# MarkTakken/kf2vecFSW

Hardware: AMD Instinct MI355X
Metric: Gbases/s k-mer→.kf build at k=7; achieved HBM GB/s vs gfx950 peak (higher is better)
Workload: dtype u32

## Files before the change

kf2vecfsw_amd/csrc/kf_count.hip:

```cpp
#include <hip/hip_runtime.h>
#include <stdint.h>
#include <stdlib.h>

#include <mutex>

#include "kf_front.h"
#include "kf_internal.h"

namespace kf {

constexpr int kBlock = 1024;
constexpr uint32_t kWaveWeights = 20u | 17u << 8 | 11u << 16 | 6u << 24;
constexpr int kXRing = 2;

__device__ __forceinline__ void wg_span(const CountArgs& A, uint64_t& lo, uint64_t& hi) {
    const uint64_t base = A.goff[0];
    const uint64_t total = A.goff[A.n_genomes] - base;
    const uint64_t G = gridDim.x, b = blockIdx.x;
    lo = base + ((total / G * b + (total % G) * b / G) & ~(uint64_t)15);
    hi = (b + 1 == G) ? base + total : base + ((total / G * (b + 1) + (total % G) * (b + 1) / G) & ~(uint64_t)15);
}

template <int K>
struct XL {
    static constexpr uint32_t P = K >= 8 ? (1u << 17) : (2u << (2 * (K + 1)));
    static constexpr uint32_t S = K >= 8 ? (1u << 15) : (2u << (2 * K));
    static constexpr uint32_t bytes = P + S;
};
constexpr int kXChunk = 3 * kChunk;
constexpr uint32_t kHot7 = 0xC000C000u, kStep7 = 0x4000u;
constexpr uint32_t kHot8 = 0xE000E000u, kStep8 = 0x2000u;
constexpr uint32_t kHot6 = 0x80008000u, kStep6 = 0x8000u;
template <int K>
constexpr uint32_t x_hot() { return K >= 8 ? kHot8 : (K == 7 ? kHot7 : kHot6); }
template <int K>
constexpr uint32_t x_step() { return K >= 8 ? kStep8 : (K == 7 ? kStep7 : kStep6); }

__device__ __forceinline__ uint32_t k9_code_of(uint32_t i) { return ((i >> 9) << 10) | (i & 0x1FFu); }

__device__ __forceinline__ uint32_t half_one(uint32_t i) { return 1u << ((i & 1u) << 4); }

template <int B>
__device__ __forceinline__ uint32_t shl1_byte(uint32_t h, uint32_t one) {
    uint32_t r;
    if constexpr (B == 0)
        asm("v_lshlrev_b32_sdwa %0, %1, %2 dst_sel:DWORD dst_unused:UNUSED_PAD src0_sel:BYTE_0 src1_sel:DWORD"
            : "=v"(r) : "v"(h), "v"(one));
    else if constexpr (B == 1)
        asm("v_lshlrev_b32_sdwa %0, %1, %2 dst_sel:DWORD dst_unused:UNUSED_PAD src0_sel:BYTE_1 src1_sel:DWORD"
            : "=v"(r) : "v"(h), "v"(one));
    else if constexpr (B == 2)
        asm("v_lshlrev_b32_sdwa %0, %1, %2 dst_sel:DWORD dst_unused:UNUSED_PAD src0_sel:BYTE_2 src1_sel:DWORD"
            : "=v"(r) : "v"(h), "v"(one));
    else
        asm("v_lshlrev_b32_sdwa %0, %1, %2 dst_sel:DWORD dst_unused:UNUSED_PAD src0_sel:BYTE_3 src1_sel:DWORD"
            : "=v"(r) : "v"(h), "v"(one));
    return r;
}

template <int K>
__device__ __noinline__ void x_drain(uint32_t a, const uint32_t* __restrict__ code2col, uint32_t* gcounts) {
    constexpr uint32_t HOT = x_hot<K>(), STEP = x_step<K>();
    constexpr uint32_t PB = XL<K>::P;
    lds_u32* p = (lds_u32*)(uintptr_t)a;
    uint32_t cur = __hip_atomic_load(p, __ATOMIC_RELAXED, __HIP_MEMORY_SCOPE_WORKGROUP);
    while (cur & HOT) {
        const uint32_t sub = ((cur & (HOT & 0xFFFF0000u)) ? (STEP << 16) : 0u) | ((cur & (HOT & 0xFFFFu)) ? STEP : 0u);
        uint32_t seen = cur;
        if (__hip_atomic_compare_exchange_strong(p, &seen, cur - sub, __ATOMIC_RELAXED, __ATOMIC_RELAXED,
                                                 __HIP_MEMORY_SCOPE_WORKGROUP)) {
            const bool single = a >= PB;
            const uint32_t w = (single ? a - PB : a) >> 2;
            for (uint32_t h = 0; h < 2; ++h) {
                if (!((sub >> (16 * h)) & 0xFFFFu)) continue;
                const uint32_t bin = 2 * w + h;
                if (K == 8 || single) {
                    atomicAdd(gcounts + code2col[bin], STEP);
                } else {
                    atomicAdd(gcounts + code2col[bin >> 2], STEP);
                    atomicAdd(gcounts + code2col[bin & ((1u << (2 * K)) - 1u)], STEP);
                }
            }
            cur -= sub;
        } else {
            cur = seen;
        }
    }
}
template <int K>
__device__ __noinline__ void x_scan_drain(const uint32_t* __restrict__ code2col, uint32_t* gcounts, int lane) {
    constexpr uint32_t HOT = x_hot<K>();
    for (uint32_t w = (uint32_t)lane; w < (K >= 8 ? XL<K>::P : XL<K>::bytes) / 4; w += kWave) {
        const uint32_t v = __hip_atomic_load((lds_u32*)(uintptr_t)(4 * w), __ATOMIC_RELAXED,
                                             __HIP_MEMORY_SCOPE_WORKGROUP);
        if (v & HOT) x_drain<K>(4 * w, code2col, gcounts);
    }
}

constexpr uint32_t kXTabLo = 0x630B6102u;
constexpr uint32_t kXTabHi = 0x67000074u;

struct XBlock {
    uint4 q[3];
};
__device__ __forceinline__ uint32_t x_zmap(uint32_t x, uint32_t e, uint32_t c) {
    uint32_t r;
    asm("v_bitop3_b32 %0, %1, %2, %3 bitop3:0x38" : "=v"(r) : "v"(x), "v"(e), "v"(c));
    return r;
}

constexpr int kXNt = 2;

__device__ __forceinline__ XBlock xc_load(const uint8_t* bytes, uint64_t c0, uint32_t rel, uint32_t end_r, int lane) {
    const uint32_t rec = end_r > rel ? min(end_r - rel, (uint32_t)kXChunk) : 0u;
    const auto rs = __builtin_amdgcn_make_buffer_rsrc((void*)(bytes + c0 + rel), (short)0, (int)rec, 0x00020000);
    XBlock b;
#pragma unroll
    for (int i = 0; i < 3; ++i) {
        const auto v = __builtin_amdgcn_raw_buffer_load_b128(rs, lane * 16 + kChunk * i, 0, kXNt);
        b.q[i] = make_uint4(v[0], v[1], v[2], v[3]);
    }
    return b;
}

__device__ __forceinline__ constexpr uint32_t xc_nl_weights(int i) {
    return (uint32_t)(64 - 8 * i) | (uint32_t)(62 - 8 * i) << 8 | (uint32_t)(60 - 8 * i) << 16 |
           (uint32_t)(58 - 8 * i) << 24;
}
constexpr uint32_t kXcBad = 68u;

struct XcCls {
    uint32_t C, V;
};
__device__ __forceinline__ XcCls xc_cls(const uint4 d) {
    const uint32_t w[4] = {d.x, d.y, d.z, d.w};
    const uint32_t cdf = 0xDFDFDFDFu;
    uint32_t pc[4], z[4];
#pragma unroll
    for (int i = 0; i < 4; ++i) {
        const uint32_t x = w[i];
        const uint32_t e = __builtin_amdgcn_perm(kXTabHi, kXTabLo, x & 0x07070707u);
        z[i] = x_zmap(x, e, cdf);
        pc[i] = __builtin_amdgcn_udot4(x & 0x06060606u, 0x01041040u, (i & 1) ? pc[i - 1] << 8 : 0u, false);
    }
    XcCls r;
    r.C = (pc[1] << 15) | (pc[3] >> 1);
    r.V = __builtin_amdgcn_udot4(z[1], xc_nl_weights(1), __builtin_amdgcn_udot4(z[0], xc_nl_weights(0), 0u, false),
                                 false) +
          __builtin_amdgcn_udot4(z[3], xc_nl_weights(3), __builtin_amdgcn_udot4(z[2], xc_nl_weights(2), 0u, false),
                                 false);
    return r;
}

struct XcWin {
    uint32_t x0, y0, c, nl;
};
__device__ __forceinline__ XcWin xc_window(const XcCls& k, uint32_t rot) {
    uint32_t nl;
    asm("v_min_u32_e32 %0, 1, %1" : "=v"(nl) : "v"(k.V));
    const uint32_t q = min(k.V - 34u, 32u);
    const uint32_t L = (uint32_t)(~0ull << q);
    const uint32_t c = bfi(L, k.C >> 2, k.C);
    const uint32_t pC = wave_shr1(rot, c);
    XcWin x;
    x.x0 = (c << 1) | ((pC << 31) & (0u - nl));
    x.y0 = (c >> 15) | (pC << (17u - 2u * nl));
    x.c = c, x.nl = nl;
    return x;
}
__device__ __forceinline__ uint32_t wave_ror1(uint32_t v) {
    return (uint32_t)__builtin_amdgcn_update_dpp(0, (int)v, 0x13C, 0xF, 0xF, false);
}

template <int K>
__device__ __forceinline__ void xc_pairs(const XcWin& x, uint32_t (&rt)[8]) {
    static_assert(K >= 2 && K <= 7, "pairs of k-mers: k <= 7");
    constexpr uint32_t PM = (1u << (2 * K + 3)) - 4u, SM = (1u << (2 * K + 1)) - 4u;
    const uint32_t one = 1u;
    const uint32_t x0 = x.x0, y0 = x.y0;
    const uint32_t H0 = (x.c << 4) & 0x10101010u, H1 = x.c & 0x10101010u;
#pragma unroll
    for (int j = 0; j < 7; ++j) {
// ... 40 lines not shown
};
__device__ __forceinline__ K9Win k9_window(const XcCls& k, uint32_t rot) {
    uint32_t nl;
    asm("v_min_u32_e32 %0, 1, %1" : "=v"(nl) : "v"(k.V));
    const uint32_t q = min(k.V - 34u, 32u);
    const uint32_t L = (uint32_t)(~0ull << q);
    const uint32_t c = bfi(L, k.C >> 2, k.C);
    const uint32_t pC = wave_shr1(rot, c);
    K9Win x;
    x.c = c, x.nl = nl;
    x.wlo = c | ((pC << 30) & (0u - nl));
    x.whi = pC >> (2u * nl);
    return x;
}

__device__ __forceinline__ uint32_t k9_index(uint32_t wlo, uint32_t whi, uint32_t rlo, uint32_t rhi, int r) {
    const uint32_t y = r < 8 ? wlo >> (2 * r) : __builtin_amdgcn_alignbit(whi, wlo, 2 * r);
    const uint32_t rc = r < 8 ? rhi >> (14 - 2 * r) : __builtin_amdgcn_alignbit(rhi, rlo, 46 - 2 * r);
    const uint32_t c = bfi((uint32_t)__builtin_amdgcn_sbfe((int)y, 9u, 1u), rc, y);
    return bfi(0x1FFu, c, c >> 1) & 0x1FFFFu;
}

__device__ __noinline__ uint32_t k9b_carries(uint32_t wlo, uint32_t whi, const uint32_t* __restrict__ code2col,
                                             uint32_t* gcounts, uint32_t w0, uint32_t w1, uint32_t w2, uint32_t w3,
                                             uint32_t w4, uint32_t w5, uint32_t w6, uint32_t w7, uint32_t w8,
                                             uint32_t w9, uint32_t w10, uint32_t w11, uint32_t w12, uint32_t w13,
                                             uint32_t w14, uint32_t w15) {
    const uint32_t rlo = revpairs(whi) ^ 0xAAAAAAAAu, rhi = revpairs(wlo) ^ 0xAAAAAAAAu;
    const uint32_t rt[16] = {w0, w1, w2, w3, w4, w5, w6, w7, w8, w9, w10, w11, w12, w13, w14, w15};
    uint32_t fixed = 0;
#pragma unroll
    for (int r = 0; r < 16; ++r) {
        const uint32_t w = rt[r], ki = k9_index(wlo, whi, rlo, rhi, r), b = ki & 3u;
        if (((w >> (8 * b)) & 0xFFu) != 0xFFu) continue;
        const uint32_t base = ki & ~3u;
        fixed = 1;
        atomicAdd(gcounts + code2col[k9_code_of(base | b)], 256u);
        for (uint32_t j = b + 1; j < 4; ++j) {
            const uint32_t col = code2col[k9_code_of(base | j)];
            const bool wraps = ((w >> (8 * j)) & 0xFFu) == 0xFFu;
            atomicAdd(gcounts + col, wraps ? 255u : 0xFFFFFFFFu);
            if (!wraps) break;
        }
    }
    return __builtin_amdgcn_ballot_w64(fixed != 0) != 0 ? 1u : 0u;
}

template <bool DENSE>
__device__ __forceinline__ uint32_t k9b_region(uint32_t wlo, uint32_t whi, uint32_t R, const CountArgs& A,
                                               uint32_t* gcounts) {
    const uint32_t rlo = revpairs(whi) ^ 0xAAAAAAAAu, rhi = revpairs(wlo) ^ 0xAAAAAAAAu;
    uint32_t rt[16];
#pragma unroll
    for (int r = 0; r < 16; ++r) {
        const uint32_t ki = k9_index(wlo, whi, rlo, rhi, r);
        rt[r] = 0;
        const bool v = (DENSE && r < 15) || ((R >> r) & 1u);
        if (v) rt[r] = lds_add_rtn(ki & 0x1FFFCu, 1u << ((ki << 3) & 24u));
    }
    uint32_t acc = 0;
#pragma unroll
    for (int r = 0; r < 16; ++r) acc |= ~(rt[r] + 0x01010101u) & rt[r];
    if (__builtin_amdgcn_ballot_w64((acc & 0x80808080u) != 0) == 0) return 0;
    return k9b_carries(wlo, whi, A.code2col, gcounts, rt[0], rt[1], rt[2], rt[3], rt[4], rt[5], rt[6], rt[7], rt[8],
                       rt[9], rt[10], rt[11], rt[12], rt[13], rt[14], rt[15]);
}

template <int K>
__device__ __forceinline__ bool xc_fast(const XBlock& d, const CountArgs& A, int lane, uint32_t& carry,
                                        uint32_t* gcounts, uint32_t& lane_total, uint32_t& drained) {
    constexpr uint32_t HOT = x_hot<K>();
    constexpr uint32_t TM = (1u << (2 * (K - 1))) - 1u;
    const XcCls k0 = xc_cls(d.q[0]), k1 = xc_cls(d.q[1]), k2 = xc_cls(d.q[2]);
    carry = __builtin_amdgcn_readfirstlane(carry);
    if (t_n(carry) < (uint32_t)(K - 1) || __builtin_amdgcn_ballot_w64(max(max(k0.V, k1.V), k2.V) >= kXcBad) != 0)
        return false;
    if constexpr (K == 9) {
        const K9Win x0 = k9_window(k0, t_codes(carry));
        uint32_t f = k9b_region<true>(x0.wlo, x0.whi, 0xFFFFu >> x0.nl, A, gcounts);
        const K9Win x1 = k9_window(k1, wave_ror1(x0.c));
        f |= k9b_region<true>(x1.wlo, x1.whi, 0xFFFFu >> x1.nl, A, gcounts);
        const K9Win x2 = k9_window(k2, wave_ror1(x1.c));
        f |= k9b_region<true>(x2.wlo, x2.whi, 0xFFFFu >> x2.nl, A, gcounts);
        lane_total -= x0.nl + x1.nl + x2.nl;
        carry = tail_pack((uint32_t)__builtin_amdgcn_readlane((int)x2.c, kWave - 1) & TM, 31u, 31u);
        drained |= f;
        return true;
    }
    uint32_t o = 0;
    const XcWin x0 = xc_window(k0, t_codes(carry));
    const XcWin x1 = xc_window(k1, wave_ror1(x0.c));
    const XcWin x2 = xc_window(k2, wave_ror1(x1.c));
    if constexpr (K <= 7) {
        const XcWin* xs[3] = {&x0, &x1, &x2};
#pragma unroll
        for (int i = 0; i < 3; ++i) {
            uint32_t r[8];
            xc_pairs<K>(*xs[i], r);
#pragma unroll
            for (int j = 0; j < 8; j += 4) o |= r[j] | r[j + 1] | r[j + 2] | r[j + 3];
        }
    } else {
        const XcWin* xs[3] = {&x0, &x1, &x2};
#pragma unroll
        for (int i = 0; i < 3; ++i) {
            uint32_t r[16];
            xc_wins8(*xs[i], r);
#pragma unroll
            for (int j = 0; j < 16; j += 4) o |= r[j] | r[j + 1] | r[j + 2] | r[j + 3];
        }
    }
    lane_total -= x0.nl + x1.nl + x2.nl;
    carry = tail_pack((uint32_t)__builtin_amdgcn_readlane((int)x2.c, kWave - 1) & TM, 31u, 31u);
    if (__builtin_amdgcn_ballot_w64((o & HOT) != 0) != 0) {
        x_scan_drain<K>(A.code2col, gcounts, lane);
        drained = 1;
    }
    return true;
}

template <int K, bool MASKED>
__device__ __forceinline__ uint32_t x_singles(const uint4 d, const CountArgs& A, uint64_t chunk, int lane,
                                              const ChunkMask& m, uint64_t iv0, uint32_t carry, uint32_t* gcounts,
                                              uint32_t& lane_total, uint32_t& drained) {
    constexpr uint32_t HOT = x_hot<K>();
    uint32_t C, V, EN, ne, own;
    front_end<K, MASKED, false>(d, A, chunk, lane, m, iv0, C, V, EN, ne, own);
    const Windows win = windows<K, MASKED>(C, V, EN, ne, carry, lane);
    const uint32_t wlo = win.wlo, whi = win.whi, R = win.R;
    if constexpr (K == 9) {
        drained |= k9b_region<false>(wlo, whi, R, A, gcounts);
        lane_total += (uint32_t)__builtin_popcount(R);
        return win.next;
    }
    const uint32_t wv[4] = {wlo, __builtin_amdgcn_alignbit(whi, wlo, 8), __builtin_amdgcn_alignbit(whi, wlo, 16),
                            __builtin_amdgcn_alignbit(whi, wlo, 24)};
    uint32_t o = 0;
#pragma unroll
    for (int r = 0; r < 16; ++r) {
        const int fo = (2 * r) & ~7;
        const uint32_t y = __builtin_amdgcn_ubfe(wv[fo >> 3], 2 * r - fo, 2 * K);
        o |= lds_add_rtn((K == 8 ? 0u : XL<K>::P) + ((y >> 1) << 2), ((R >> r) & 1u) * half_one(y));
    }
    if (__builtin_amdgcn_ballot_w64((o & HOT) != 0) != 0) {
        x_scan_drain<K>(A.code2col, gcounts, lane);
        drained = 1;
    }
    lane_total += (uint32_t)__builtin_popcount(R);
    return win.next;
}

template <int K>
__device__ __forceinline__ uint32_t x_range(const CountArgs& A, int32_t g, uint64_t glo, uint64_t ghi, uint64_t lo,
                                            uint64_t hi, int lane, uint32_t& drained) {
    if (lo >= hi) return 0;
    uint32_t* gcounts = A.counts + (uint64_t)g * A.nbins;
    Range rg;
    rg.init(glo, ghi, lo, hi);
    auto load = [&](uint32_t r) {
        return xc_load(A.bytes, rg.c0, r, rg.end_r, lane);
    };
    static_assert(kXRing == 2, "two-deep register ring");
    XBlock buf[K == 9 ? 1 : kXRing];
    XBlock b0, b1;
    if constexpr (K == 9) {
        b0 = load(0);
        b1 = load(kXChunk);
    } else {
#pragma unroll
        for (int j = 0; j < kXRing; ++j) buf[j] = load(j * kXChunk);
    }
    const uint32_t nx = (rg.nch + 2) / 3;
    rg.warm16<K>(A, lane);
    __builtin_amdgcn_s_setprio(0);
    uint32_t carry = rg.carry;
    uint32_t rel = 0;
    const ChunkMask m = rg.mask();
    uint32_t lane_total = 0;
    uint32_t nfast = 0;
    auto step = [&](const XBlock& bf) {
        bool fast = !rg.masked_span(A, rel, kXChunk);
        if (fast)
            fast = xc_fast<K>(bf, A, lane, carry, gcounts, lane_total, drained);
        nfast += fast ? 1u : 0u;
        if (!fast) {
            const bool m0 = rg.masked(A, rel);
            const uint64_t iv0 = rg.iv;
            const bool m1 = rg.masked(A, rel + kChunk);
            const uint64_t iv1 = rg.iv;
            const bool m2 = rg.masked(A, rel + 2 * kChunk);
#pragma unroll
            for (int h = 0; h < 3; ++h) {
                const uint32_t r = rel + h * kChunk;
                if (h > 0 && r >= rg.nch * kChunk) break;
                const bool mh = h == 0 ? m0 : (h == 1 ? m1 : m2);
                const uint64_t ivh = h == 0 ? iv0 : (h == 1 ? iv1 : rg.iv);
                const uint4 hb = bf.q[h];
                if (mh)
                    carry = x_singles<K, true>(hb, A, rg.c0 + r, lane, m, ivh, carry, gcounts, lane_total, drained);
                else
                    carry = x_singles<K, false>(hb, A, rg.c0 + r, lane, m, ivh, carry, gcounts, lane_total, drained);
            }
        }
        rel += kXChunk;
    };
    if constexpr (K == 9) {
        for (uint32_t i = 0; i + 2 <= nx; i += 2) {
            step(b0);
            b0 = load(rel + kXChunk);
            step(b1);
            b1 = load(rel + kXChunk);
        }
        if (nx & 1u) step(b0);
    } else {
        for (uint32_t i = 0; i + kXRing <= nx; i += kXRing) {
#pragma unroll
            for (int j = 0; j < kXRing; ++j) {
                step(buf[j]);
                buf[j] = load(rel + (kXRing - 1) * kXChunk);
            }
        }
        const uint32_t rem = nx % kXRing;
#pragma unroll
        for (int j = 0; j < kXRing - 1; ++j)
            if (rem > (uint32_t)j) step(buf[j]);
    }
    return lane_total + 48u * nfast;
}

__device__ __forceinline__ uint32_t f_swz(uint32_t y) { return y ^ (((y >> 8) & 15u) << 1); }
__device__ __forceinline__ uint32_t u16sum2(uint32_t w) { return (w & 0xFFFFu) + (w >> 16); }

__device__ __forceinline__ void pair_f_sums(const uint32_t* hist, int tid, uint32_t (&F)[16]) {
    const uint4* h4 = (const uint4*)hist;
#pragma unroll
    for (int i = 0; i < 8; ++i) {
        const uint4 w = h4[i * 1024 + tid];
        F[2 * i] = u16sum2(w.x) + u16sum2(w.y);
        F[2 * i + 1] = u16sum2(w.z) + u16sum2(w.w);
#pragma unroll
        for (int a = 0; a < 4; ++a) {
            const uint32_t v = hist[a * 8192 + i * 1024 + tid];
            F[2 * i] += v & 0xFFFFu;
            F[2 * i + 1] += v >> 16;
        }
    }
}

template <int K>
__device__ __forceinline__ void pair_f_sums_small(const uint32_t* hist, int tid,
                                                  uint32_t (&F)[((1u << (2 * K)) + kBlock - 1) / kBlock]) {
    constexpr uint32_t NY = 1u << (2 * K), NM = (NY + kBlock - 1) / kBlock;
#pragma unroll
    for (uint32_t m = 0; m < NM; ++m) {
        const uint32_t y = (uint32_t)tid + kBlock * m;
        F[m] = 0;
        if (y < NY) {
            const uint32_t sh = (y & 1u) << 4;
            uint32_t f = u16sum2(hist[2 * y]) + u16sum2(hist[2 * y + 1]);
#pragma unroll
            for (uint32_t a = 0; a < 4; ++a) f += (hist[a * (NY / 2) + (y >> 1)] >> sh) & 0xFFFFu;
            f += (hist[XL<K>::P / 4 + (y >> 1)] >> sh) & 0xFFFFu;
            F[m] = f;
        }
    }
}

template <int K>
__global__ void __launch_bounds__(kBlock) __attribute__((amdgpu_waves_per_eu(4, 4))) k1x_kernel(CountArgs A) {
    static_assert(K >= 2 && K <= 9, "K1x serves k = 2 .. 9 (k = 9: K9b byte counters)");
    extern __shared__ __attribute__((aligned(16))) uint32_t hist[];
    const int tid = threadIdx.x;
    const int lane = tid & (kWave - 1);
    const int wave = __builtin_amdgcn_readfirstlane(tid >> 6);
    {
        uint4* h4 = (uint4*)hist;
        for (uint32_t i = tid; i < XL<K>::bytes / 16; i += kBlock) h4[i] = make_uint4(0u, 0u, 0u, 0u);
    }
    __syncthreads();
    if ((uint32_t)(uintptr_t)(lds_u32*)hist != 0u) __builtin_trap();
    uint64_t span_lo, span_hi;
    wg_span(A, span_lo, span_hi);
    if (span_lo >= span_hi) return;
    int32_t g = (int32_t)wave_upper_bound((uint64_t)A.n_genomes, span_lo, lane,
                                          [&](uint64_t i) { return A.goff[i + 1]; });
    const uint32_t fr_lo = wave_frac((uint32_t)wave, kWaveWeights), fr_hi = wave_frac((uint32_t)wave + 1, kWaveWeights);
    for (; g < A.n_genomes; ++g) {
        __builtin_amdgcn_s_setprio(3);
        const uint64_t glo = A.goff[g], ghi = A.goff[g + 1];
        if (glo >= span_hi) break;
        const uint64_t plo = max(glo, span_lo), phi = min(ghi, span_hi);
        if (phi <= plo) continue;
        const uint64_t lo = split_at_frac(plo, phi, fr_lo), hi = split_at_frac(plo, phi, fr_hi);
        uint32_t drained = 0;
        unsigned long long s = x_range<K>(A, g, glo, ghi, lo, hi, lane, drained);
        uint32_t* gc = A.counts + (uint64_t)g * A.nbins;
        const bool whole = plo == glo && phi == ghi && !(A.flags & KF_ACCUMULATE);
        if constexpr (K == 9) {
            lds_barrier();
            if (lane == 0) hist[XL<K>::P / 4 + wave] = drained;
            lds_barrier();
            const uint4* fl = (const uint4*)(hist + XL<K>::P / 4);
            const uint4 f0 = fl[0], f1 = fl[1], f2 = fl[2], f3 = fl[3];
            const bool any_fix = (f0.x | f0.y | f0.z | f0.w | f1.x | f1.y | f1.z | f1.w | f2.x | f2.y | f2.z |
                                  f2.w | f3.x | f3.y | f3.z | f3.w) != 0;
            const uint8_t* hb = (const uint8_t*)hist;
            for (uint32_t c0 = (uint32_t)tid; c0 < (1u << 17); c0 += 4 * kBlock) {
                uint32_t rep[4];
#pragma unroll
                for (int j = 0; j < 4; ++j) rep[j] = A.col2rep[c0 + j * kBlock];
#pragma unroll
                for (int j = 0; j < 4; ++j) {
                    const uint32_t c = (rep[j] & 0x200u) ? kf_revcomp<9>(rep[j]) : rep[j];
                    const uint32_t v = hb[((c >> 1) & 0x1FE00u) | (c & 0x1FFu)];
                    if (whole && !any_fix)
                        __builtin_nontemporal_store(v, gc + c0 + j * kBlock);
                    else if (v)
                        __hip_atomic_fetch_add(gc + c0 + j * kBlock, v, __ATOMIC_RELAXED, __HIP_MEMORY_SCOPE_AGENT);
                }
            }
            lds_barrier();
            uint4* h4 = (uint4*)hist;
            for (uint32_t i = tid; i < XL<K>::bytes / 16; i += kBlock) h4[i] = make_uint4(0u, 0u, 0u, 0u);
        } else if constexpr (K == 8) {
            lds_barrier();
            if (lane == 0) hist[XL<K>::P / 4 + wave] = drained;
            lds_barrier();
            const uint4* fl = (const uint4*)(hist + XL<K>::P / 4);
            const uint4 f0 = fl[0], f1 = fl[1], f2 = fl[2], f3 = fl[3];
            const bool any_drain = (f0.x | f0.y | f0.z | f0.w | f1.x | f1.y | f1.z | f1.w | f2.x | f2.y | f2.z |
                                    f2.w | f3.x | f3.y | f3.z | f3.w) != 0;
            for (uint32_t col = tid; col < A.nbins; col += kBlock) {
                const uint32_t y = A.col2rep[col], rc = kf_revcomp<8>(y);
                uint32_t v = (hist[y >> 1] >> ((y & 1u) << 4)) & 0xFFFFu;
                if (rc != y) v += (hist[rc >> 1] >> ((rc & 1u) << 4)) & 0xFFFFu;
                if (whole && !any_drain)
                    gc[col] = v;
                else if (v)
                    __hip_atomic_fetch_add(gc + col, v, __ATOMIC_RELAXED, __HIP_MEMORY_SCOPE_AGENT);
            }
            lds_barrier();
            uint4* h4 = (uint4*)hist;
            for (uint32_t i = tid; i < XL<K>::bytes / 16; i += kBlock) h4[i] = make_uint4(0u, 0u, 0u, 0u);
        } else if constexpr (K <= 6) {
            constexpr uint32_t NY = 1u << (2 * K), NM = (NY + kBlock - 1) / kBlock;
            constexpr uint32_t NCOL = (NY + (K % 2 == 0 ? (1u << K) : 0u)) / 2, NC = (NCOL + kBlock - 1) / kBlock;
            uint32_t rep[NC];
#pragma unroll
            for (uint32_t c = 0; c < NC; ++c) {
                const uint32_t col = (uint32_t)tid + c * kBlock;
                rep[c] = col < NCOL ? A.col2rep[col] : 0u;
            }
            lds_barrier();
            uint32_t F[NM];
            pair_f_sums_small<K>(hist, tid, F);
            lds_barrier();
#pragma unroll
            for (uint32_t m = 0; m < NM; ++m) {
                const uint32_t y = (uint32_t)tid + kBlock * m;
                if (y < NY) hist[f_swz(y)] = F[m];
            }
            if (lane == 0) hist[NY + wave] = drained;
            lds_barrier();
            const uint4* fl = (const uint4*)(hist + NY);
            const uint4 f0 = fl[0], f1 = fl[1], f2 = fl[2], f3 = fl[3];
            const bool any_drain = (f0.x | f0.y | f0.z | f0.w | f1.x | f1.y | f1.z | f1.w | f2.x | f2.y | f2.z | f2.w |
                                    f3.x | f3.y | f3.z | f3.w) != 0;
            uint32_t cv[NC];
#pragma unroll
            for (uint32_t c = 0; c < NC; ++c) {
                const uint32_t y = rep[c], rc = kf_revcomp<K>(y);
                cv[c] = hist[f_swz(y)] + (rc != y ? hist[f_swz(rc)] : 0u);
            }
            lds_barrier();
            uint4* h4 = (uint4*)hist;
            for (uint32_t i = tid; i < XL<K>::bytes / 16; i += kBlock) h4[i] = make_uint4(0u, 0u, 0u, 0u);
#pragma unroll
            for (uint32_t c = 0; c < NC; ++c) {
                const uint32_t col = (uint32_t)tid + c * kBlock;
                if (col >= NCOL) continue;
                if (whole && !any_drain)
                    __builtin_nontemporal_store(cv[c], gc + col);
                else if (cv[c])
                    __hip_atomic_fetch_add(gc + col, cv[c], __ATOMIC_RELAXED, __HIP_MEMORY_SCOPE_AGENT);
            }
        } else {
            uint32_t rep[8];
            if (whole) {
                const uint4 r0 = *(const uint4*)(A.col2rep + 4 * tid), r1 = *(const uint4*)(A.col2rep + 4096 + 4 * tid);
                rep[0] = r0.x, rep[1] = r0.y, rep[2] = r0.z, rep[3] = r0.w;
                rep[4] = r1.x, rep[5] = r1.y, rep[6] = r1.z, rep[7] = r1.w;
            } else {
#pragma unroll
                for (int c = 0; c < 8; ++c) rep[c] = A.col2rep[tid + c * kBlock];
            }
            lds_barrier();
            uint32_t F[16];
            pair_f_sums(hist, tid, F);
#pragma unroll
            for (int i = 0; i < 8; ++i) {
                const uint32_t v = hist[XL<K>::P / 4 + i * 1024 + tid];
                F[2 * i] += v & 0xFFFFu;
                F[2 * i + 1] += v >> 16;
            }
            lds_barrier();
#pragma unroll
            for (int i = 0; i < 8; ++i) *(uint2*)(hist + f_swz(i * 2048 + 2 * tid)) = make_uint2(F[2 * i], F[2 * i + 1]);
            if (lane == 0) hist[16384 + wave] = drained;
            lds_barrier();
            const uint4* fl = (const uint4*)(hist + 16384);
            const uint4 f0 = fl[0], f1 = fl[1], f2 = fl[2], f3 = fl[3];
            const bool any_drain = (f0.x | f0.y | f0.z | f0.w | f1.x | f1.y | f1.z | f1.w | f2.x | f2.y | f2.z | f2.w |
                                    f3.x | f3.y | f3.z | f3.w) != 0;
            uint32_t cv[8];
#pragma unroll
            for (int c = 0; c < 8; ++c) {
                const uint32_t y = rep[c], rc = kf_revcomp<7>(y);
                cv[c] = hist[f_swz(y)] + hist[f_swz(rc)];
            }
            lds_barrier();
            uint4* h4 = (uint4*)hist;
            for (uint32_t i = tid; i < XL<K>::bytes / 16; i += kBlock) h4[i] = make_uint4(0u, 0u, 0u, 0u);
            if (whole && !any_drain) {
                typedef unsigned int v4u_t __attribute__((ext_vector_type(4)));
                __builtin_nontemporal_store(v4u_t{cv[0], cv[1], cv[2], cv[3]}, (v4u_t*)(gc + 4 * tid));
                __builtin_nontemporal_store(v4u_t{cv[4], cv[5], cv[6], cv[7]}, (v4u_t*)(gc + 4096 + 4 * tid));
            } else {
#pragma unroll
                for (int c = 0; c < 8; ++c) {
                    const uint32_t col = whole ? (c >> 2) * 4096 + 4 * tid + (c & 3) : tid + c * kBlock;
                    if (cv[c]) __hip_atomic_fetch_add(gc + col, cv[c], __ATOMIC_RELAXED, __HIP_MEMORY_SCOPE_AGENT);
                }
            }
        }
        s = wave_sum(s);
        if (lane == 0 && s) atomicAdd(A.totals + g, s);
        lds_barrier();
    }
}

__device__ __forceinline__ uint64_t splitmix64(uint64_t x) {
    x += 0x9E3779B97F4A7C15ull;
    x = (x ^ (x >> 30)) * 0xBF58476D1CE4E5B9ull;
    x = (x ^ (x >> 27)) * 0x94D049BB133111EBull;
    return x ^ (x >> 31);
}

__device__ __forceinline__ bool in_nrun(uint64_t key, uint64_t i, uint64_t n_period) {
    if (!n_period) return false;
    uint64_t b = i >> 12;
    for (int d = 0; d < 2; ++d) {
        if (d == 1) {
            if (b == 0) break;
            b -= 1;
        }
        const uint64_t h = splitmix64((key ^ 0xA5A5A5A5A5A5A5A5ull) + b);
        if (h % n_period) continue;
        const uint64_t st = (b << 12) + ((h >> 16) % 4096), ln = 1 + ((h >> 32) % 100);
        if (i >= st && i < st + ln) return true;
    }
    return false;
}

__global__ void __launch_bounds__(256) synth_kernel(uint8_t* bytes, const uint64_t* goff, int64_t g0, int64_t gstride,
                                                     uint64_t seed0, uint64_t seq_len, int width, uint64_t n_period) {
    const int32_t gi = blockIdx.y;
    const uint64_t lo = goff[gi], hi = goff[gi + 1];
    const int64_t g = g0 + gi * gstride;
    char digits[24];
    int nd = 0;
    {
        uint64_t v = (uint64_t)(g < 0 ? -g : g);
        do { digits[nd++] = (char)('0' + v % 10); v /= 10; } while (v);
    }
    const uint64_t hlen = 5 + (uint64_t)nd + (g < 0 ? 1 : 0) + 1;
    const uint64_t key = splitmix64(seed0 + (uint64_t)g);
    const uint64_t W1 = (uint64_t)width + 1;
    for (uint64_t p0 = ((uint64_t)blockIdx.x * blockDim.x + threadIdx.x) * 16; lo + p0 < hi;
         p0 += (uint64_t)gridDim.x * blockDim.x * 16) {
        uint32_t out[4] = {0, 0, 0, 0};
        for (int j = 0; j < 16; ++j) {
            const uint64_t p = p0 + j;
            uint32_t ch;
            if (p < hlen) {
                if (p == 0) ch = '>';
                else if (p < 5) ch = "syn_"[p - 1];
                else if (g < 0 && p == 5) ch = '-';
                else if (p == hlen - 1) ch = '\n';
                else ch = (uint32_t)digits[nd - 1 - (int)(p - 5 - (g < 0 ? 1 : 0))];
            } else {
                const uint64_t q = p - hlen, line = q / W1, col = q % W1;
                const uint64_t i = line * (uint64_t)width + col;
                if (col == (uint64_t)width || i >= seq_len) {
                    ch = '\n';
                } else {
                    const uint64_t h = splitmix64(key + (i >> 5));
                    ch = (uint32_t)"ACGT"[(h >> (2 * (i & 31))) & 3];
                    if (in_nrun(key, i, n_period)) ch = 'N';
                }
            }
            out[j >> 2] |= ch << (8 * (j & 3));
        }
        if (lo + p0 + 16 <= hi) {
            *(uint4*)(bytes + lo + p0) = make_uint4(out[0], out[1], out[2], out[3]);
        } else {
            for (int j = 0; lo + p0 + j < hi; ++j) bytes[lo + p0 + j] = (uint8_t)(out[j >> 2] >> (8 * (j & 3)));
        }
    }
}

__device__ __forceinline__ uint32_t wave_xor(uint32_t v) {
#pragma unroll
    for (int d = 1; d < kWave; d <<= 1) v ^= (uint32_t)__shfl_xor((int)v, d, kWave);
    return v;
}

__global__ void __launch_bounds__(1024) stream_probe_kernel(const uint8_t* bytes, uint64_t n, uint32_t* out) {
    const int lane = threadIdx.x & (kWave - 1);
    const uint64_t nw = (uint64_t)gridDim.x * (blockDim.x / kWave);
    const uint64_t w = (uint64_t)blockIdx.x * (blockDim.x / kWave) + (threadIdx.x >> 6);
    constexpr uint32_t kB = 3 * kChunk;
    const uint64_t nblk = (n + kB - 1) / kB;
    uint32_t acc = 0;
    for (uint64_t b = w; b < nblk; b += 4 * nw) {
        uint4 v[4][3];
#pragma unroll
        for (int k = 0; k < 4; ++k) {
            const uint64_t bb = b + (uint64_t)k * nw;
            const uint64_t base = bb < nblk ? bb * kB : 0;
            const int rec = bb < nblk ? (int)min((uint64_t)kB, n - base) : 0;
            const auto rs = __builtin_amdgcn_make_buffer_rsrc((void*)(bytes + base), (short)0, rec, 0x00020000);
#pragma unroll
            for (int q = 0; q < 3; ++q) {
                const auto t = __builtin_amdgcn_raw_buffer_load_b128(rs, 16 * lane + 1024 * q, 0, 0);
                v[k][q] = make_uint4(t[0], t[1], t[2], t[3]);
            }
        }
#pragma unroll
        for (int k = 0; k < 4; ++k)
#pragma unroll
            for (int q = 0; q < 3; ++q) acc ^= v[k][q].x ^ v[k][q].y ^ v[k][q].z ^ v[k][q].w;
    }
    acc = wave_xor(acc);
    if (lane == 0 && acc) atomicXor(out, acc);
}

}

using namespace kf;

namespace {

void* kernel_for(int k) {
    switch (k) {
    case 2: return (void*)&k1x_kernel<2>;
    case 3: return (void*)&k1x_kernel<3>;
    case 4: return (void*)&k1x_kernel<4>;
    case 5: return (void*)&k1x_kernel<5>;
    case 6: return (void*)&k1x_kernel<6>;
    case 7: return (void*)&k1x_kernel<7>;
    case 8: return (void*)&k1x_kernel<8>;
    case 9: return (void*)&k1x_kernel<9>;
    default: return nullptr;
    }
}

int lds_bytes_for(int k) {
    switch (k) {
    case 2: return (int)XL<2>::bytes;
    case 3: return (int)XL<3>::bytes;
    case 4: return (int)XL<4>::bytes;
    case 5: return (int)XL<5>::bytes;
    case 6: return (int)XL<6>::bytes;
    case 7: return (int)XL<7>::bytes;
    case 8: return (int)XL<8>::bytes;
// ... 118 lines not shown
```

kf2vecfsw_amd/csrc/kf_front.h:

```cpp
#pragma once
#include <hip/hip_runtime.h>
#include <stdint.h>

#include "kf_scan.h"

namespace kf {

constexpr int kWave = 64;
constexpr int kChunk = 1024;

struct CountArgs {
    const uint8_t* bytes;
    const uint64_t* goff;
    const uint64_t* excl;
    uint64_t n_excl;
    const uint32_t* code2col;
    const uint32_t* col2rep;
    uint32_t* counts;
    unsigned long long* totals;
    uint32_t nbins;
    int32_t n_genomes;
    uint32_t flags;
};

// ... 54 lines not shown
        const uint32_t z = (x ^ ex) & 0xDFDFDFDFu;
        nf[q] = __builtin_amdgcn_perm(0xFFFFFFFFu, 0xFFFFFFFFu, x ^ 0x06060606u);
        bad |= z & nf[q];
        pc[q] = __builtin_amdgcn_udot4(cb, 0x01041040u, 0u, false);
    }
    const uint32_t c01 = __builtin_amdgcn_perm(pc[0], pc[1], 0x0C0C0400u);
    const uint32_t c23 = __builtin_amdgcn_perm(pc[2], pc[3], 0x0C0C0400u);
    C = (c01 << 16) | c23;
    auto pair = [](const uint32_t a, const uint32_t b) -> uint32_t {
        return (uint32_t)__builtin_amdgcn_sdot4((int)a, (int)0xF0E0C080u,
                                               __builtin_amdgcn_sdot4((int)b, (int)0xFFFEFCF8u, 0, false), false);
    };
    NNL = (pair(nf[0], nf[1]) << 8) | pair(nf[2], nf[3]);
}

__device__ __forceinline__ uint32_t bfi(uint32_t m, uint32_t a, uint32_t b) { return (m & a) | (~m & b); }

template <bool MASKED>
__device__ __forceinline__ void remove_entry(uint32_t r, uint32_t& C, uint32_t& V, uint32_t& EN, uint32_t& nl) {
    const uint32_t lo1 = (1u << r) - 1u;
    const uint32_t lo2 = lo1 | (lo1 << r);
    V = bfi(lo1, V, V >> 1);
    if (MASKED) EN = bfi(lo1, EN, EN >> 1);
    C = bfi(lo2, C, C >> 2);
    nl = (nl >> 1) & ~lo1;
}

template <bool MASKED>
__device__ __forceinline__ void compact(uint32_t nl, uint32_t& C, uint32_t& V, uint32_t& EN) {
    remove_entry<MASKED>((uint32_t)__builtin_ctz(nl | 0x10000u), C, V, EN, nl);
    while (nl) remove_entry<MASKED>((uint32_t)__builtin_ctz(nl), C, V, EN, nl);
}

__device__ __forceinline__ uint32_t revpairs(uint32_t x) {
    const uint32_t t = __builtin_bitreverse32(x);
    return ((t << 1) & 0xAAAAAAAAu) | ((t >> 1) & 0x55555555u);
}

template <int K>
__device__ __forceinline__ uint32_t kf_revcomp(uint32_t x) {
    return (revpairs(x) >> (32 - 2 * K)) ^ (0xAAAAAAAAu >> (32 - 2 * K));
}

template <int K>
__device__ __forceinline__ uint32_t run_mask(uint32_t E) {
    uint32_t R = E;
    int a = 1;
#pragma unroll
    for (int it = 0; it < 5; ++it) {
        if (a < K) {
            const int s = (a < K - a) ? a : (K - a);
            R &= R >> s;
            a += s;
        }
    }
    return R;
}

__device__ __forceinline__ uint32_t wave_shr1(uint32_t old, uint32_t v) {
    return (uint32_t)__builtin_amdgcn_update_dpp((int)old, (int)v, 0x138, 0xF, 0xF, false);
}

template <int K>
__device__ __noinline__ uint32_t scan_ctx(uint32_t own, uint32_t carry, int lane) {
    uint32_t v = own;
#pragma unroll
    for (int d = 1; d < kWave; d <<= 1) {
        const uint32_t o = __shfl_up(v, d, kWave);
        if (lane >= d) v = tail_combine<K>(o, v);
    }
    const uint32_t ex = __shfl_up(v, 1, kWave);
    return lane == 0 ? carry : tail_combine<K>(carry, ex);
}

__device__ __forceinline__ uint64_t uload64(const uint64_t* p) {
    const uint64_t v = *p;
    return ((uint64_t)__builtin_amdgcn_readfirstlane((uint32_t)(v >> 32)) << 32) |
           (uint64_t)__builtin_amdgcn_readfirstlane((uint32_t)v);
}

struct ChunkMask {
    uint64_t glo;
    uint64_t lo;
    uint64_t hi;
};

__device__ __forceinline__ uint32_t range_bits(int64_t a, int64_t b) {
    a = a < 0 ? 0 : (a > 16 ? 16 : a);
    b = b < 0 ? 0 : (b > 16 ? 16 : b);
    if (b <= a) return 0u;
    const uint32_t n = (uint32_t)(b - a);
    return ((n >= 32 ? 0xFFFFFFFFu : ((1u << n) - 1u)) << (16 - (uint32_t)b)) & 0xFFFFu;
}

__device__ __forceinline__ void apply_masks(const CountArgs& A, uint64_t chunk, int lane,
                                            const ChunkMask& m, uint64_t iv0,
                                            uint32_t& INV, uint32_t& EN) {
    const int64_t b0 = (int64_t)(chunk + 16u * (uint32_t)lane);
    INV |= range_bits(-1, (int64_t)m.glo - b0);
    EN = range_bits((int64_t)m.lo - b0, (int64_t)m.hi - b0);
    const uint64_t cend = chunk + kChunk;
    for (uint64_t i = iv0; i < A.n_excl; ++i) {
        const uint64_t s = uload64(A.excl + 2 * i), e = uload64(A.excl + 2 * i + 1);
        if (s >= cend) break;
        INV |= range_bits((int64_t)s - b0, (int64_t)e - b0);
    }
}

constexpr int kChunkCpol = 2;
__device__ __forceinline__ uint4 load_chunk(const uint8_t* bytes, uint64_t c0, uint32_t rel, uint32_t end_r,
                                            int lane) {
    const uint32_t rec = end_r > rel ? min(end_r - rel, (uint32_t)kChunk) : 0u;
    const auto rs = __builtin_amdgcn_make_buffer_rsrc((void*)(bytes + c0 + rel), (short)0, (int)rec, 0x00020000);
    const auto v = __builtin_amdgcn_raw_buffer_load_b128(rs, lane * 16, 0, kChunkCpol);
    return make_uint4(v[0], v[1], v[2], v[3]);
}

template <int K>
__device__ __forceinline__ uint32_t own_tail(uint32_t C, uint32_t V, uint32_t ne) {
    constexpr uint32_t TM = (K > 1) ? ((1u << (2 * (K - 1))) - 1u) : 0u;
    return (C & TM) | ((uint32_t)__builtin_ctz(~V) << 22) | (ne << 27);
}

template <int K, bool MASKED, bool OWN = true>
__device__ __forceinline__ void front_end(const uint4 d, const CountArgs& A, uint64_t chunk, int lane,
                                          const ChunkMask& m, uint64_t iv0,
                                          uint32_t& C, uint32_t& V, uint32_t& EN, uint32_t& ne,
                                          uint32_t& own) {
    uint32_t INV, NNL;
    classify16(d, C, INV, NNL);
    EN = 0xFFFFu;
    if (MASKED) apply_masks(A, chunk, lane, m, iv0, INV, EN);
    V = ~INV & 0xFFFFu;
    ne = (uint32_t)__builtin_popcount(NNL);
    compact<MASKED>(NNL ^ 0xFFFFu, C, V, EN);
    if (OWN) own = own_tail<K>(C, V, ne);
}

template <class KeyF>
__device__ __forceinline__ uint64_t wave_upper_bound(uint64_t n, uint64_t x, int lane, KeyF key) {
    uint64_t a = 0, b = n;
    while (b - a > (uint64_t)kWave) {
        const uint64_t step = (b - a + kWave - 1) / kWave;
        const uint64_t i = a + step * (uint64_t)lane;
        const uint32_t cnt = (uint32_t)__builtin_popcountll(__ballot(i < b && key(i) <= x));
        const uint64_t na = cnt ? a + step * (cnt - 1) + 1 : a;
        b = min(b, a + step * cnt);
        a = na;
    }
    const uint64_t i = a + (uint64_t)lane;
    return a + (uint64_t)__builtin_popcountll(__ballot(i < b && key(i) <= x));
}

__device__ __forceinline__ uint4 chunk_tail_load(const uint8_t* bytes, int64_t p, uint64_t glo, int lane) {
    const int64_t b0 = p + 16 * lane;
    uint4 d = make_uint4(0u, 0u, 0u, 0u);
    if (b0 >= (int64_t)(glo & ~(uint64_t)15)) d = *(const uint4*)(bytes + b0);
    return d;
}

template <int K>
__device__ __noinline__ uint32_t chunk_tail_data(const uint4 d, const uint8_t* bytes, const uint64_t* excl,
                                                 uint64_t n_excl, int64_t p, uint64_t glo, int lane) {
    CountArgs A{};
    A.bytes = bytes;
    A.excl = excl;
    A.n_excl = n_excl;
    const uint64_t key = p < 0 ? 0 : (uint64_t)p;
    const uint64_t lo = wave_upper_bound(A.n_excl, key, lane, [&](uint64_t i) { return A.excl[2 * i + 1]; });
    ChunkMask m{glo, 0, 0};
    uint32_t C, V, EN, ne, own;
    front_end<K, true>(d, A, (uint64_t)p, lane, m, lo, C, V, EN, ne, own);
    uint32_t v = own;
#pragma unroll
    for (int dd = 1; dd < kWave; dd <<= 1) {
        const uint32_t o = __shfl_up(v, dd, kWave);
        if (lane >= dd) v = tail_combine<K>(o, v);
    }
    return (uint32_t)__builtin_amdgcn_readlane((int)v, kWave - 1);
}

template <int K>
__device__ __forceinline__ uint32_t chunk_tail(const uint8_t* bytes, const uint64_t* excl, uint64_t n_excl, int64_t p,
                                               uint64_t glo, int lane) {
    return chunk_tail_data<K>(chunk_tail_load(bytes, p, glo, lane), bytes, excl, n_excl, p, glo, lane);
}


struct Range {
    uint64_t c0, glo, ghi, lo, hi;
    uint32_t lo_r, hi_r, end_r, nch;
    uint64_t iv;
    uint32_t ivs_r, ive_r;
    uint64_t ivs_a, ive_a;
    uint32_t carry;

    __device__ __forceinline__ uint32_t rel_of(uint64_t x) const {
        return x <= c0 ? 0u : (x - c0 >= 0xFFFFFFFFull ? 0xFFFFFFFFu : (uint32_t)(x - c0));
    }
    __device__ __forceinline__ void init(uint64_t glo_, uint64_t ghi_, uint64_t lo_, uint64_t hi_) {
        glo = glo_, ghi = ghi_, lo = lo_, hi = hi_;
        c0 = lo & ~(uint64_t)15;
        lo_r = (uint32_t)(lo - c0);
        hi_r = (uint32_t)(hi - c0);
        end_r = rel_of((ghi + 15) & ~(uint64_t)15);
        nch = (hi_r + kChunk - 1) / kChunk;
    }
    template <int K>
    __device__ __forceinline__ void warm(const CountArgs& A, int lane) {
        carry = tail_pack(0, 0, 0);
        for (int64_t p = (int64_t)c0; p > (int64_t)glo && !tail_complete<K>(carry);) {
            p -= kChunk;
            carry = tail_combine<K>(chunk_tail<K>(A.bytes, A.excl, A.n_excl, p, glo, lane), carry);
        }
        find_interval(A, lane);
    }
    template <int K>
    __device__ __forceinline__ void warm16(const CountArgs& A, int lane) {
        if (c0 < glo + 16) {
            warm<K>(A, lane);
            return;
        }
        const uint64_t p16 = c0 - 16;
        const uint4 d = *(const uint4*)(A.bytes + p16);
        uint64_t s_iv = ~0ull, e_iv = ~0ull;
        iv = wave_upper_bound(A.n_excl, p16, lane, [&](uint64_t i) { return A.excl[2 * i + 1]; });
        if (iv < A.n_excl) {
            s_iv = uload64(A.excl + 2 * iv);
            e_iv = uload64(A.excl + 2 * iv + 1);
        }
        uint32_t C, V, EN, ne, own;
        const ChunkMask m{glo, 0, 0};
        front_end<K, false>(d, A, p16, lane, m, iv, C, V, EN, ne, own);
        if (s_iv < c0 || t_n(own) < (uint32_t)(K - 1)) {
            warm<K>(A, lane);
            return;
        }
        carry = own;
        ivs_r = iv < A.n_excl ? rel_of(s_iv) : 0xFFFFFFFFu;
        ive_r = iv < A.n_excl ? rel_of(e_iv) : 0xFFFFFFFFu;
        ivs_a = s_iv, ive_a = e_iv;
    }
    __device__ __forceinline__ void find_interval(const CountArgs& A, int lane) {
        iv = wave_upper_bound(A.n_excl, c0, lane, [&](uint64_t i) { return A.excl[2 * i + 1]; });
        ivs_r = ive_r = 0xFFFFFFFFu;
        ivs_a = ive_a = ~0ull;
        if (iv < A.n_excl) {
            ivs_a = uload64(A.excl + 2 * iv);
            ive_a = uload64(A.excl + 2 * iv + 1);
            ivs_r = rel_of(ivs_a);
            ive_r = rel_of(ive_a);
        }
    }
    __device__ __forceinline__ bool masked(const CountArgs& A, uint32_t rel) {
        if (rel >= ive_r) {
            const uint64_t cc = c0 + rel;
            do { ++iv; } while (iv < A.n_excl && uload64(A.excl + 2 * iv + 1) <= cc);
            ivs_a = iv < A.n_excl ? uload64(A.excl + 2 * iv) : ~0ull;
            ive_a = iv < A.n_excl ? uload64(A.excl + 2 * iv + 1) : ~0ull;
            ivs_r = iv < A.n_excl ? rel_of(ivs_a) : 0xFFFFFFFFu;
            ive_r = iv < A.n_excl ? rel_of(ive_a) : 0xFFFFFFFFu;
        }
        return ivs_r < rel + kChunk || rel < lo_r || rel + kChunk > hi_r;
    }
    __device__ __forceinline__ bool masked_span(const CountArgs& A, uint32_t rel, uint32_t len) {
        if (rel >= ive_r) return masked(A, rel) || ivs_r < rel + len || rel + len > hi_r;
        return ivs_r < rel + len || rel < lo_r || rel + len > hi_r;
    }
    __device__ __forceinline__ ChunkMask mask() const { return ChunkMask{glo, lo, hi}; }
    __device__ __forceinline__ uint4 load(const uint8_t* bytes, uint32_t rel, int lane) const {
        return load_chunk(bytes, c0, rel, end_r, lane);
    }
};

__device__ __forceinline__ uint64_t split_at(uint64_t plo, uint64_t phi, uint64_t w, uint64_t n) {
    if (w == 0) return plo;
    if (w >= n) return phi;
    const uint64_t len = phi - plo;
    const uint64_t s = (plo + len / n * w + (len % n) * w / n) & ~(uint64_t)15;
    return min(max(s, plo), phi);
}

__device__ __forceinline__ uint32_t wave_frac(uint32_t w, uint32_t wts) {
    if (w == 0) return 0u;
    if (w >= 16) return 1u << 20;
    const uint32_t b0 = wts & 0xFFu, b1 = (wts >> 8) & 0xFFu, b2 = (wts >> 16) & 0xFFu, b3 = wts >> 24;
    const uint32_t tot = 4u * (b0 + b1 + b2 + b3);
    const uint32_t s = w >> 2, r = w & 3u;
    uint32_t cum = 0;
    cum += (s > 0 ? 4u * b0 : (r ? r * b0 : 0u));
    cum += (s > 1 ? 4u * b1 : (s == 1 ? r * b1 : 0u));
    cum += (s > 2 ? 4u * b2 : (s == 2 ? r * b2 : 0u));
    cum += (s == 3 ? r * b3 : 0u);
    return (cum << 20) / tot;
}

__device__ __forceinline__ uint64_t split_at_frac(uint64_t plo, uint64_t phi, uint32_t fr) {
    if (fr >= (1u << 20)) return phi;
    const uint64_t x = (plo + (((phi - plo) * fr) >> 20)) & ~(uint64_t)15;
    return min(max(x, plo), phi);
}

struct Windows {
    uint32_t wlo, whi, R, next;
};
template <int K, bool MASKED>
__device__ __forceinline__ Windows windows(uint32_t C, uint32_t V, uint32_t EN, uint32_t ne, uint32_t carry,
                                           int lane) {
    constexpr uint32_t TM = (K > 1) ? ((1u << (2 * (K - 1))) - 1u) : 0u;
    const uint32_t own = own_tail<K>(C, V, ne);
    uint32_t ctx = wave_shr1(carry, own);
    if (__ballot(ne < (uint32_t)(K - 1)) != 0) {
        const uint64_t inc_mask = __ballot(!tail_complete<K>(own)) & 0x7FFFFFFFFFFFFFFFull;
        if (inc_mask) ctx = scan_ctx<K>(own, carry, lane);
    }
    const uint64_t W = ((uint64_t)t_codes(ctx) << (2 * ne)) | (uint64_t)C;
    Windows w;
    w.wlo = (uint32_t)W;
    w.whi = (uint32_t)(W >> 32);
    const uint32_t ctxlen = min(t_n(ctx), (uint32_t)(K - 1));
    const uint32_t E = (((1u << ctxlen) - 1u) << ne) | V;
    w.R = run_mask<K>(E) & ((1u << ne) - 1u);
    if (MASKED) w.R &= EN;
    const uint32_t incl = tail_pack(w.wlo & TM, (uint32_t)__builtin_ctz(~E), 31u);
    w.next = (uint32_t)__builtin_amdgcn_readlane((int)incl, kWave - 1);
    return w;
}

__device__ __forceinline__ unsigned long long wave_sum(unsigned long long v) {
#pragma unroll
    for (int d = 32; d >= 1; d >>= 1) v += __shfl_xor(v, d, kWave);
    return v;
}

int bucket_launch(const CountArgs& A, int k, uint32_t flags, hipStream_t s);
int bucket_launch_info(int k, int* grid, int* block, int* lds);
int bucket_reserve(int k, int32_t max_genomes);

}
```

Measured before the change: 5735.

## Split wave ranges on chunk lattice, hint interval search, prefetch genome offsets

Wave sub-ranges within a genome are now split on whole 3-chunk iteration boundaries, so waves avoid partial ragged iterations. The exclusion-interval lookup in warm-up reuses a per-wave hint with a one-wave ballot scan instead of a full binary search. Genome offsets are prefetched one genome ahead. LDS zeroing of the unused table region is moved before the barrier so it overlaps the flag exchange. This adds some complexity and relies on kLattice matching kXChunk.

```diff
diff --git a/kf2vecfsw_amd/csrc/kf_count.hip b/kf2vecfsw_amd/csrc/kf_count.hip
--- a/kf2vecfsw_amd/csrc/kf_count.hip
+++ b/kf2vecfsw_amd/csrc/kf_count.hip
@@ -28,6 +28,8 @@
     static constexpr uint32_t bytes = P + S;
 };
 constexpr int kXChunk = 3 * kChunk;
+static_assert((uint32_t)kXChunk == kLattice, "wave ranges are split on the iteration lattice (split_at_lattice)");
+constexpr uint32_t kLatticeMaxIters = 2560;
 constexpr uint32_t kHot7 = 0xC000C000u, kStep7 = 0x4000u;
 constexpr uint32_t kHot8 = 0xE000E000u, kStep8 = 0x2000u;
 constexpr uint32_t kHot6 = 0x80008000u, kStep6 = 0x8000u;
@@ -374,7 +376,7 @@
 
 template <int K>
 __device__ __forceinline__ uint32_t x_range(const CountArgs& A, int32_t g, uint64_t glo, uint64_t ghi, uint64_t lo,
-                                            uint64_t hi, int lane, uint32_t& drained) {
+                                            uint64_t hi, int lane, uint64_t& iv_hint, uint32_t& drained) {
     if (lo >= hi) return 0;
     uint32_t* gcounts = A.counts + (uint64_t)g * A.nbins;
     Range rg;
@@ -393,7 +395,7 @@
         for (int j = 0; j < kXRing; ++j) buf[j] = load(j * kXChunk);
     }
     const uint32_t nx = (rg.nch + 2) / 3;
-    rg.warm16<K>(A, lane);
+    rg.warm16<K>(A, lane, iv_hint);
     __builtin_amdgcn_s_setprio(0);
     uint32_t carry = rg.carry;
     uint32_t rel = 0;
@@ -488,6 +490,11 @@
     }
 }
 
+__device__ __forceinline__ void lds_zero(uint32_t* hist, uint32_t lo4, uint32_t hi4, int tid) {
+    uint4* h4 = (uint4*)hist;
+    for (uint32_t i = lo4 + (uint32_t)tid; i < hi4; i += kBlock) h4[i] = make_uint4(0u, 0u, 0u, 0u);
+}
+
 template <int K>
 __global__ void __launch_bounds__(kBlock) __attribute__((amdgpu_waves_per_eu(4, 4))) k1x_kernel(CountArgs A) {
     static_assert(K >= 2 && K <= 9, "K1x serves k = 2 .. 9 (k = 9: K9b byte counters)");
@@ -507,15 +514,21 @@
     int32_t g = (int32_t)wave_upper_bound((uint64_t)A.n_genomes, span_lo, lane,
                                           [&](uint64_t i) { return A.goff[i + 1]; });
     const uint32_t fr_lo = wave_frac((uint32_t)wave, kWaveWeights), fr_hi = wave_frac((uint32_t)wave + 1, kWaveWeights);
+    uint64_t g_lo = A.goff[g], g_hi = A.goff[g + 1];
+    uint64_t iv_hint = 0;
     for (; g < A.n_genomes; ++g) {
         __builtin_amdgcn_s_setprio(3);
-        const uint64_t glo = A.goff[g], ghi = A.goff[g + 1];
+        const uint64_t glo = g_lo, ghi = g_hi;
+        g_lo = g_hi;
+        g_hi = A.goff[min(g + 2, A.n_genomes)];
         if (glo >= span_hi) break;
         const uint64_t plo = max(glo, span_lo), phi = min(ghi, span_hi);
         if (phi <= plo) continue;
-        const uint64_t lo = split_at_frac(plo, phi, fr_lo), hi = split_at_frac(plo, phi, fr_hi);
+        const uint32_t nit = lattice_iters(plo, phi);
+        const bool lat = nit <= kLatticeMaxIters;
+        const uint64_t lo = split_at_lattice(plo, phi, nit, lat, fr_lo), hi = split_at_lattice(plo, phi, nit, lat, fr_hi);
         uint32_t drained = 0;
-        unsigned long long s = x_range<K>(A, g, glo, ghi, lo, hi, lane, drained);
+        unsigned long long s = x_range<K>(A, g, glo, ghi, lo, hi, lane, iv_hint, drained);
         uint32_t* gc = A.counts + (uint64_t)g * A.nbins;
         const bool whole = plo == glo && phi == ghi && !(A.flags & KF_ACCUMULATE);
         if constexpr (K == 9) {
@@ -567,6 +580,8 @@
         } else if constexpr (K <= 6) {
             constexpr uint32_t NY = 1u << (2 * K), NM = (NY + kBlock - 1) / kBlock;
             constexpr uint32_t NCOL = (NY + (K % 2 == 0 ? (1u << K) : 0u)) / 2, NC = (NCOL + kBlock - 1) / kBlock;
+            constexpr uint32_t ZF = (NY + 16) / 4;
+            static_assert(ZF <= XL<K>::bytes / 16, "F and the flags lie inside the table");
             uint32_t rep[NC];
 #pragma unroll
             for (uint32_t c = 0; c < NC; ++c) {
@@ -583,6 +598,7 @@
                 if (y < NY) hist[f_swz(y)] = F[m];
             }
             if (lane == 0) hist[NY + wave] = drained;
+            lds_zero(hist, ZF, XL<K>::bytes / 16, tid);
             lds_barrier();
             const uint4* fl = (const uint4*)(hist + NY);
             const uint4 f0 = fl[0], f1 = fl[1], f2 = fl[2], f3 = fl[3];
@@ -595,8 +611,7 @@
                 cv[c] = hist[f_swz(y)] + (rc != y ? hist[f_swz(rc)] : 0u);
             }
             lds_barrier();
-            uint4* h4 = (uint4*)hist;
-            for (uint32_t i = tid; i < XL<K>::bytes / 16; i += kBlock) h4[i] = make_uint4(0u, 0u, 0u, 0u);
+            lds_zero(hist, 0, ZF, tid);
 #pragma unroll
             for (uint32_t c = 0; c < NC; ++c) {
                 const uint32_t col = (uint32_t)tid + c * kBlock;
@@ -629,6 +644,8 @@
 #pragma unroll
             for (int i = 0; i < 8; ++i) *(uint2*)(hist + f_swz(i * 2048 + 2 * tid)) = make_uint2(F[2 * i], F[2 * i + 1]);
             if (lane == 0) hist[16384 + wave] = drained;
+            constexpr uint32_t ZF = (16384 + 16) / 4;
+            lds_zero(hist, ZF, XL<K>::bytes / 16, tid);
             lds_barrier();
             const uint4* fl = (const uint4*)(hist + 16384);
             const uint4 f0 = fl[0], f1 = fl[1], f2 = fl[2], f3 = fl[3];
@@ -641,8 +658,7 @@
                 cv[c] = hist[f_swz(y)] + hist[f_swz(rc)];
             }
             lds_barrier();
-            uint4* h4 = (uint4*)hist;
-            for (uint32_t i = tid; i < XL<K>::bytes / 16; i += kBlock) h4[i] = make_uint4(0u, 0u, 0u, 0u);
+            lds_zero(hist, 0, ZF, tid);
             if (whole && !any_drain) {
                 typedef unsigned int v4u_t __attribute__((ext_vector_type(4)));
                 __builtin_nontemporal_store(v4u_t{cv[0], cv[1], cv[2], cv[3]}, (v4u_t*)(gc + 4 * tid));
diff --git a/kf2vecfsw_amd/csrc/kf_front.h b/kf2vecfsw_amd/csrc/kf_front.h
--- a/kf2vecfsw_amd/csrc/kf_front.h
+++ b/kf2vecfsw_amd/csrc/kf_front.h
@@ -230,6 +230,35 @@
     return a + (uint64_t)__builtin_popcountll(__ballot(i < b && key(i) <= x));
 }
 
+struct IvHit {
+    uint64_t iv, s, e;
+};
+__device__ __forceinline__ uint64_t readlane64(uint64_t v, uint32_t l) {
+    return ((uint64_t)(uint32_t)__builtin_amdgcn_readlane((int)(uint32_t)(v >> 32), (int)l) << 32) |
+           (uint64_t)(uint32_t)__builtin_amdgcn_readlane((int)(uint32_t)v, (int)l);
+}
+__device__ __forceinline__ IvHit interval_after(const CountArgs& A, uint64_t x, uint64_t hint, int lane) {
+    const uint64_t i = hint + (uint64_t)lane;
+    uint64_t s = ~0ull, e = ~0ull;
+    if (i < A.n_excl) s = A.excl[2 * i], e = A.excl[2 * i + 1];
+    const uint32_t cnt = (uint32_t)__builtin_popcountll(__ballot(e <= x));
+    IvHit r;
+    if (cnt < (uint32_t)kWave) {
+        r.iv = hint + cnt;
+        r.s = readlane64(s, cnt);
+        r.e = readlane64(e, cnt);
+        return r;
+    }
+    const uint64_t a = hint + kWave;
+    r.iv = a + wave_upper_bound(A.n_excl - a, x, lane, [&](uint64_t j) { return A.excl[2 * (a + j) + 1]; });
+    r.s = r.e = ~0ull;
+    if (r.iv < A.n_excl) {
+        r.s = uload64(A.excl + 2 * r.iv);
+        r.e = uload64(A.excl + 2 * r.iv + 1);
+    }
+    return r;
+}
+
 __device__ __forceinline__ uint4 chunk_tail_load(const uint8_t* bytes, int64_t p, uint64_t glo, int lane) {
     const int64_t b0 = p + 16 * lane;
     uint4 d = make_uint4(0u, 0u, 0u, 0u);
@@ -294,30 +323,40 @@
         find_interval(A, lane);
     }
     template <int K>
-    __device__ __forceinline__ void warm16(const CountArgs& A, int lane) {
+    __device__ __forceinline__ void warm16(const CountArgs& A, int lane, uint64_t& hint) {
         if (c0 < glo + 16) {
-            warm<K>(A, lane);
+            warm_hinted<K>(A, lane, hint);
             return;
         }
         const uint64_t p16 = c0 - 16;
         const uint4 d = *(const uint4*)(A.bytes + p16);
-        uint64_t s_iv = ~0ull, e_iv = ~0ull;
-        iv = wave_upper_bound(A.n_excl, p16, lane, [&](uint64_t i) { return A.excl[2 * i + 1]; });
-        if (iv < A.n_excl) {
-            s_iv = uload64(A.excl + 2 * iv);
-            e_iv = uload64(A.excl + 2 * iv + 1);
-        }
+        const IvHit h = interval_after(A, p16, hint, lane);
+        iv = hint = h.iv;
+        const uint64_t s_iv = h.s, e_iv = h.e;
         uint32_t C, V, EN, ne, own;
         const ChunkMask m{glo, 0, 0};
         front_end<K, false>(d, A, p16, lane, m, iv, C, V, EN, ne, own);
         if (s_iv < c0 || t_n(own) < (uint32_t)(K - 1)) {
-            warm<K>(A, lane);
+            warm_hinted<K>(A, lane, hint);
             return;
         }
         carry = own;
         ivs_r = iv < A.n_excl ? rel_of(s_iv) : 0xFFFFFFFFu;
         ive_r = iv < A.n_excl ? rel_of(e_iv) : 0xFFFFFFFFu;
         ivs_a = s_iv, ive_a = e_iv;
+    }
+    template <int K>
+    __device__ __forceinline__ void warm_hinted(const CountArgs& A, int lane, uint64_t& hint) {
+        carry = tail_pack(0, 0, 0);
+        for (int64_t p = (int64_t)c0; p > (int64_t)glo && !tail_complete<K>(carry);) {
+            p -= kChunk;
+            carry = tail_combine<K>(chunk_tail<K>(A.bytes, A.excl, A.n_excl, p, glo, lane), carry);
+        }
+        const IvHit h = interval_after(A, c0, hint, lane);
+        iv = hint = h.iv;
+        ivs_a = h.s, ive_a = h.e;
+        ivs_r = iv < A.n_excl ? rel_of(ivs_a) : 0xFFFFFFFFu;
+        ive_r = iv < A.n_excl ? rel_of(ive_a) : 0xFFFFFFFFu;
     }
     __device__ __forceinline__ void find_interval(const CountArgs& A, int lane) {
         iv = wave_upper_bound(A.n_excl, c0, lane, [&](uint64_t i) { return A.excl[2 * i + 1]; });
@@ -379,6 +418,18 @@
     return min(max(x, plo), phi);
 }
 
+constexpr uint32_t kLattice = 3 * kChunk;
+__device__ __forceinline__ uint32_t lattice_iters(uint64_t plo, uint64_t phi) {
+    return (uint32_t)((phi - (plo & ~(uint64_t)15) + (kLattice - 1)) >> 10) / (kLattice >> 10);
+}
+__device__ __forceinline__ uint64_t split_at_lattice(uint64_t plo, uint64_t phi, uint32_t nit, bool lat, uint32_t fr) {
+    if (fr == 0) return plo;
+    if (fr >= (1u << 20)) return phi;
+    const uint64_t m = ((lat ? (uint64_t)nit : phi - plo) * fr + (lat ? 1u << 19 : 0u)) >> 20;
+    const uint64_t x = lat ? (plo & ~(uint64_t)15) + m * kLattice : (plo + m) & ~(uint64_t)15;
+    return min(max(x, plo), phi);
+}
+
 struct Windows {
     uint32_t wlo, whi, R, next;
 };
```

Result: faster. 5837 (median of 6 runs) (+1.8%).
